# aanna0701/face-recognition-pytorch

Measured on AMD Instinct MI355X. Metric: train imgs/sec IR-50-layout ResNet50 + ArcFace/PartialFC head, 112x112, higher is better.
Workload: dtype bf16

## Files before the change

### face-recognition-pytorch_amd/frhip/build.py

```python
import hashlib
import os
import subprocess
import sys

HERE = os.path.dirname(os.path.abspath(__file__))
CSRC = os.path.join(HERE, "csrc")
ROOT = os.path.dirname(os.path.dirname(HERE))
LIB = os.path.join(HERE, "libfrhip.so")
SOURCES = ["misc.hip", "bn.hip", "stem.hip", "stem_fused.hip", "stem_algebra.hip", "igemm_nt.hip", "igemm_halo.hip", "igemm_tn.hip", "igemm_fp8.hip", "head.hip", "pfc_sample.hip", "margin.hip", "gallery_topk.hip", "winattn.hip", "winattn_mfma.hip", "cpb.hip", "optim.hip", "augment.hip"]
HIPCC = os.environ.get("HIPCC", "/opt/rocm/bin/hipcc")
FLAGS = ["--offload-arch=gfx950", "-O3", "-fPIC", "-std=c++17", "-munsafe-fp-atomics",
         "-I" + os.path.join(ROOT, "include"), "-I" + CSRC]
VARIANT = os.environ.get("FRHIP_VARIANT", "")
if VARIANT:
    FLAGS = FLAGS + os.environ.get("FRHIP_CXXFLAGS", "").split()
    LIB = os.path.join(HERE, "build", "var", "libfrhip_%s.so" % VARIANT)


def _digest(paths):
    h = hashlib.sha1(" ".join(FLAGS).replace(ROOT, "").encode())
    for p in sorted(paths):
        h.update(os.path.basename(p).encode())
        with open(p, "rb") as f:
            h.update(f.read())
    return h.hexdigest()


def _stale(target, deps):
    stamp = target + ".sha1"
    if not os.path.exists(target) or not os.path.exists(stamp):
        return True
    with open(stamp) as f:
        return f.read().strip() != _digest(deps)


def build(force=False, verbose=False):
    objdir = os.path.join(HERE, "build", "var", VARIANT) if VARIANT else os.path.join(HERE, "build")
    os.makedirs(objdir, exist_ok=True)
    headers = [os.path.join(CSRC, f) for f in os.listdir(CSRC) if f.endswith(".h")]
    headers.append(os.path.join(ROOT, "include", "frhip.h"))
    objs, procs = [], []
    for src in SOURCES:
        s = os.path.join(CSRC, src)
        o = os.path.join(objdir, src.replace(".hip", ".o"))
        objs.append(o)
        if force or _stale(o, [s] + headers):
            cmd = [HIPCC] + FLAGS + ["-c", s, "-o", o]
            if verbose:
                print(" ".join(cmd))
            procs.append((src, o, [s] + headers, subprocess.Popen(cmd, stdout=subprocess.PIPE, stderr=subprocess.STDOUT)))
    for src, o, deps, p in procs:
        out, _ = p.communicate()
        if p.returncode != 0:
            raise RuntimeError("hipcc failed on %s:\n%s" % (src, out.decode(errors="replace")))
        with open(o + ".sha1", "w") as f:
            f.write(_digest(deps))
    if force or procs or not os.path.exists(LIB):
        cmd = [HIPCC, "--offload-arch=gfx950", "-shared", "-fPIC", "-o", LIB] + objs
        r = subprocess.run(cmd, stdout=subprocess.PIPE, stderr=subprocess.STDOUT)
        if r.returncode != 0:
            raise RuntimeError("link failed:\n" + r.stdout.decode(errors="replace"))
    return LIB


if __name__ == "__main__":
    print(build(force="--force" in sys.argv, verbose=True))
```

### face-recognition-pytorch_amd/frhip/csrc/stem_algebra.hip

```cpp
#include "common.h"
#include "frhip.h"

namespace frhip {

constexpr int SG_ROWS = 8;
constexpr int SG_ROLES = 8;
constexpr int SG_VALS = 81;
constexpr int SG_OUT = 7 * SG_VALS;

template <typename T>
__global__ __launch_bounds__(256) void stem_gram_kernel(const float* __restrict__ x, float* __restrict__ partial, int B, int H, int W) {
    extern __shared__ __attribute__((aligned(16))) char smem[];
    float* xs = reinterpret_cast<float*>(smem);
    const int XR = SG_ROWS + 2, XC = W + 2;
    const int role = threadIdx.x & 7, pl = threadIdx.x >> 3;
    const int ca_ = role < 3 ? 0 : (role < 5 ? 1 : 2);
    const int cb_ = role < 3 ? role : (role < 5 ? role - 2 : 2);
    float acc[SG_VALS];
#pragma unroll
    for (int i = 0; i < SG_VALS; ++i) acc[i] = 0.f;
    const int bands = (H + SG_ROWS - 1) / SG_ROWS;
    for (int tile = blockIdx.x; tile < B * bands; tile += gridDim.x) {
        const int n = tile / bands, h0 = (tile - n * bands) * SG_ROWS;
        const float* ximg = x + (size_t)n * 3 * H * W;
        __syncthreads();
        for (int idx = threadIdx.x; idx < 3 * XR * XC; idx += 256) {
            const int cc = idx % XC, rest = idx / XC, rr = rest % XR, ci = rest / XR;
            const int h = h0 - 1 + rr, w = cc - 1;
            const float v = ((unsigned)h < (unsigned)H && (unsigned)w < (unsigned)W) ? ximg[((size_t)ci * H + h) * W + w] : 0.f;
            xs[idx] = to_f32<T>(from_f32<T>(v));
        }
        __syncthreads();
        const int rows = min(SG_ROWS, H - h0);
        for (int p = pl; p < rows * W; p += 32) {
            const int py = p / W, px = p - py * W;
            const float* base = xs + py * XC + px;
            if (role < 6) {
                float va[9], vb[9];
#pragma unroll
                for (int a = 0; a < 9; ++a) {
                    va[a] = base[(ca_ * XR + a / 3) * XC + a % 3];
                    vb[a] = base[(cb_ * XR + a / 3) * XC + a % 3];
                }
#pragma unroll
                for (int a = 0; a < 9; ++a)
#pragma unroll
                    for (int b = 0; b < 9; ++b) acc[a * 9 + b] = fmaf(va[a], vb[b], acc[a * 9 + b]);
            } else if (role == 6) {
#pragma unroll
                for (int c = 0; c < 3; ++c)
#pragma unroll
                    for (int a = 0; a < 9; ++a) acc[c * 9 + a] += base[(c * XR + a / 3) * XC + a % 3];
            }
        }
    }
    __syncthreads();
    float* red = reinterpret_cast<float*>(smem);
    const int lane = lane_id(), wave = wave_id();
#pragma unroll
    for (int i = 0; i < SG_VALS; ++i) {
        float v = acc[i];
        v = lane_sum_bit3(v); v = lane_sum_bit4(v); v = lane_sum_bit5(v);
        if (lane < 8) red[(wave * 8 + lane) * SG_VALS + i] = v;
    }
    __syncthreads();
    for (int o = threadIdx.x; o < SG_OUT; o += 256)
        partial[(size_t)blockIdx.x * SG_OUT + o] = red[o] + red[8 * SG_VALS + o] + red[16 * SG_VALS + o] + red[24 * SG_VALS + o];
}

__global__ __launch_bounds__(256) void stem_gram_fold_kernel(const float* __restrict__ partial, int nparts, float* __restrict__ blk) {
    __shared__ float red[3][SG_VALS];
    const int o = threadIdx.x % SG_VALS, part = threadIdx.x / SG_VALS;
    if (part < 3) {
        float a = 0.f;
        for (int p = part; p < nparts; p += 3) a += partial[(size_t)p * SG_OUT + blockIdx.x * SG_VALS + o];
        red[part][o] = a;
    }
    __syncthreads();
    if (threadIdx.x < SG_VALS) blk[blockIdx.x * SG_VALS + o] = red[0][o] + red[1][o] + red[2][o];
}

__global__ __launch_bounds__(256) void stem_gram_assemble_kernel(const float* __restrict__ blk, float* __restrict__ gram) {
    for (int o = threadIdx.x; o < 27 * 27 + 27; o += 256) {
        if (o < 729) {
            const int j = o / 27, j2 = o - j * 27;
            const int a = j / 3, c = j - a * 3, b = j2 / 3, c2 = j2 - b * 3;
            const int lo = c < c2 ? c : c2, hi = c < c2 ? c2 : c;
            const int role = lo == 0 ? hi : (lo == 1 ? 2 + hi : 5);
            gram[o] = c <= c2 ? blk[role * SG_VALS + a * 9 + b] : blk[role * SG_VALS + b * 9 + a];
        } else {
            const int j = o - 729, a = j / 3, c = j - a * 3;
            gram[o] = blk[6 * SG_VALS + c * 9 + a];
        }
    }
}

constexpr int DG_P = 8;
constexpr int DG_X = 2 * DG_P + 3;

template <typename T>
__global__ __launch_bounds__(256) void stem_dgather_kernel(const float* __restrict__ x, const T* __restrict__ dpool,
                                                           const T* __restrict__ pooled, const uint8_t* __restrict__ argmax,
                                                           float* __restrict__ slabs, int B, int H, int W) {
    __shared__ float xs[3 * DG_X * DG_X];
    __shared__ float gs[4 * 64 * 27];
    __shared__ uint8_t ab8[DG_P * DG_P * 64];
    const int Hp = (H - 1) / 2 + 1, Wp = (W - 1) / 2 + 1;
    const int th = (Hp + DG_P - 1) / DG_P, tw = (Wp + DG_P - 1) / DG_P;
    const int lane = lane_id(), wave = wave_id();
    float acc[27];
#pragma unroll
    for (int j = 0; j < 27; ++j) acc[j] = 0.f;
    constexpr int EPV = 16 / (int)sizeof(T), VPR = 64 / EPV;
    constexpr int XN = (3 * DG_X * DG_X + 255) / 256;
    constexpr int VN = DG_P * DG_P * VPR / 256;
    static_assert(DG_P * DG_P * VPR % 256 == 0, "tile vectors split evenly over the threads");
    float xr[XN];
    Vec16<T> gr[VN], pr[VN];
    uint64_t ar[VN];
    bool inr[VN];
    auto fetch = [&](int tile) {
        const int n = tile / (th * tw), rem = tile - n * th * tw;
        const int ph0 = (rem / tw) * DG_P, pw0 = (rem % tw) * DG_P;
        const float* ximg = x + (size_t)n * 3 * H * W;
#pragma unroll
        for (int i = 0; i < XN; ++i) {
            const int idx = threadIdx.x + i * 256;
            const int cc = idx % DG_X, rest = idx / DG_X, rr = rest % DG_X, ci = rest / DG_X;
            const int h = 2 * ph0 - 2 + rr, w = 2 * pw0 - 2 + cc;
            xr[i] = (idx < 3 * DG_X * DG_X && (unsigned)h < (unsigned)H && (unsigned)w < (unsigned)W) ? ximg[((size_t)ci * H + h) * W + w] : 0.f;
        }
#pragma unroll
        for (int i = 0; i < VN; ++i) {
            const int idx = threadIdx.x + i * 256;
            const int cv = idx % VPR, pp = idx / VPR, pl = pp / DG_P, pc = pp - pl * DG_P;
            const int ph = ph0 + pl, pw = pw0 + pc;
            inr[i] = ph < Hp && pw < Wp;
            const size_t o = ((((size_t)n * Hp + ph) * Wp + pw) * VPR + cv) * EPV;
            ar[i] = 0;
            if (inr[i]) {
                gr[i] = *reinterpret_cast<const Vec16<T>*>(dpool + o);
                pr[i] = *reinterpret_cast<const Vec16<T>*>(pooled + o);
                if constexpr (EPV == 8) ar[i] = *reinterpret_cast<const uint64_t*>(argmax + o);
                else ar[i] = *reinterpret_cast<const uint32_t*>(argmax + o);
            }
        }
    };
    const int ntiles = B * th * tw;
    if ((int)blockIdx.x < ntiles) fetch(blockIdx.x);
    for (int tile = blockIdx.x; tile < ntiles; tile += gridDim.x) {
        __syncthreads();
#pragma unroll
        for (int i = 0; i < XN; ++i) {
            const int idx = threadIdx.x + i * 256;
            if (idx < 3 * DG_X * DG_X) xs[idx] = to_f32<T>(from_f32<T>(xr[i]));
        }
#pragma unroll
        for (int i = 0; i < VN; ++i) {
            const int idx = threadIdx.x + i * 256;
            const int cv = idx % VPR, pp = idx / VPR;
#pragma unroll
            for (int e = 0; e < EPV; ++e) gs[pp * 64 + cv * EPV + e] = (inr[i] && pr[i].get(e) > 0.f) ? gr[i].get(e) : 0.f;
            if constexpr (EPV == 8) *reinterpret_cast<uint64_t*>(ab8 + pp * 64 + cv * 8) = ar[i];
            else *reinterpret_cast<uint32_t*>(ab8 + pp * 64 + cv * 4) = (uint32_t)ar[i];
        }
        __syncthreads();
        if (tile + (int)gridDim.x < ntiles) fetch(tile + gridDim.x);
        for (int pp = wave; pp < DG_P * DG_P; pp += 4) {
            const int pl = pp / DG_P, pc = pp - pl * DG_P;
            const float g = gs[pp * 64 + lane];
            const int a = ab8[pp * 64 + lane];
            const int r = (a * 11) >> 5, s = a - 3 * r;
            const float* base = xs + (2 * pl + r) * DG_X + 2 * pc + s;
#pragma unroll
            for (int t = 0; t < 9; ++t)
#pragma unroll
                for (int ci = 0; ci < 3; ++ci) acc[t * 3 + ci] = fmaf(g, base[(ci * DG_X + t / 3) * DG_X + t % 3], acc[t * 3 + ci]);
        }
    }
    __syncthreads();
    float* red = gs;
#pragma unroll
    for (int j = 0; j < 27; ++j) red[(wave * 64 + lane) * 27 + j] = acc[j];
    __syncthreads();
    for (int o = threadIdx.x; o < 64 * 32; o += 256) {
        const int k = o >> 5, j = o & 31;
        float a = 0.f;
        if (j < 27)
#pragma unroll
            for (int wv = 0; wv < 4; ++wv) a += red[(wv * 64 + k) * 27 + j];
        slabs[(size_t)blockIdx.x * 2048 + o] = a;
    }
}

template <typename T>
__global__ __launch_bounds__(1024) void stem_dw_final_kernel(const float* __restrict__ slabs, int nslabs, const float* __restrict__ gram,
                                                            const T* __restrict__ wp, const float* __restrict__ ca,
                                                            const float* __restrict__ cb, const float* __restrict__ cc,
                                                            float* __restrict__ dw) {
    __shared__ float red[32][32];
    const int k = blockIdx.x, j = threadIdx.x & 31, part = threadIdx.x >> 5;
    float a = 0.f;
    for (int s = part; s < nslabs; s += 32) a += slabs[(size_t)s * 2048 + k * 32 + j];
    red[part][j] = a;
    __syncthreads();
    if (threadIdx.x < 27) {
        float d = 0.f;
#pragma unroll
        for (int p = 0; p < 32; ++p) d += red[p][j];
        float wg = 0.f;
        for (int j2 = 0; j2 < 27; ++j2) wg = fmaf(to_f32<T>(wp[k * 32 + j2]), gram[j2 * 27 + j], wg);
        dw[k * 27 + j] += ca[k] * d + cb[k] * wg + cc[k] * gram[729 + j];
    }
}

}

using namespace frhip;

static bool sa_ok(int dtype, int b, int h, int w, const char* who) {
    if ((dtype != FRHIP_DT_BF16 && dtype != FRHIP_DT_F32) || b <= 0 || h <= 0 || w <= 0 || 3LL * b * h * w > 0x7fffffffLL ||
        3 * (SG_ROWS + 2) * (w + 2) * 4 > 60 * 1024) {
        set_error("%s: unsupported dtype / shape (dtype=%d b=%d h=%d w=%d)", who, dtype, b, h, w);
        return false;
    }
    return true;
}

extern "C" int frhip_stem_gram_floats(void) { return 27 * 27 + 27; }

extern "C" int frhip_stem_gram_blocks(int b, int h, int w) {
    const int t = b * ((h + SG_ROWS - 1) / SG_ROWS);
    return t < 512 ? t : 512;
}

extern "C" int frhip_stem_gram(int dtype, const float* x, int b, int h, int w, float* partial, float* gram, hipStream_t stream) {
    if (!sa_ok(dtype, b, h, w, "frhip_stem_gram")) return FRHIP_EINVAL;
    const int blocks = frhip_stem_gram_blocks(b, h, w);
    int lds = 3 * (SG_ROWS + 2) * (w + 2) * 4;
    if (lds < 4 * 8 * SG_VALS * 4) lds = 4 * 8 * SG_VALS * 4;
    if (dtype == FRHIP_DT_BF16) hipLaunchKernelGGL(stem_gram_kernel<bf16_t>, dim3(blocks), dim3(256), lds, stream, x, partial, b, h, w);
    else hipLaunchKernelGGL(stem_gram_kernel<float>, dim3(blocks), dim3(256), lds, stream, x, partial, b, h, w);
    int rc = check_launch("frhip_stem_gram");
    if (rc) return rc;
    float* blk = partial + (size_t)blocks * SG_OUT;
    hipLaunchKernelGGL(stem_gram_fold_kernel, dim3(7), dim3(256), 0, stream, partial, blocks, blk);
    hipLaunchKernelGGL(stem_gram_assemble_kernel, dim3(1), dim3(256), 0, stream, blk, gram);
    return check_launch("frhip_stem_gram(reduce)");
}

extern "C" int frhip_stem_bwd_wgrad_gram(int dtype, const float* x, const void* wp, const void* dpool, const void* pooled,
                                         const uint8_t* argmax, const float* gram, const float* ca, const float* cb, const float* cc,
                                         int b, int h, int w, float* slabs, float* dw, hipStream_t stream) {
    if (!sa_ok(dtype, b, h, w, "frhip_stem_bwd_wgrad_gram")) return FRHIP_EINVAL;
    const int blocks = frhip_stem_blocks(b, h, w);
    if (dtype == FRHIP_DT_BF16)
        hipLaunchKernelGGL(stem_dgather_kernel<bf16_t>, dim3(blocks), dim3(256), 0, stream, x, (const bf16_t*)dpool, (const bf16_t*)pooled,
                           argmax, slabs, b, h, w);
    else
        hipLaunchKernelGGL(stem_dgather_kernel<float>, dim3(blocks), dim3(256), 0, stream, x, (const float*)dpool, (const float*)pooled,
                           argmax, slabs, b, h, w);
    int rc = check_launch("frhip_stem_bwd_wgrad_gram(gather)");
    if (rc) return rc;
    if (dtype == FRHIP_DT_BF16)
        hipLaunchKernelGGL(stem_dw_final_kernel<bf16_t>, dim3(64), dim3(1024), 0, stream, slabs, blocks, gram, (const bf16_t*)wp, ca, cb, cc, dw);
    else
        hipLaunchKernelGGL(stem_dw_final_kernel<float>, dim3(64), dim3(1024), 0, stream, slabs, blocks, gram, (const float*)wp, ca, cb, cc, dw);
    return check_launch("frhip_stem_bwd_wgrad_gram(final)");
}
```

### face-recognition-pytorch_amd/frhip/csrc/stem_fused.hip

```cpp
#include "common.h"
#include "frhip.h"

namespace frhip {

constexpr int SF_PH = 4, SF_PW = 28;
constexpr int SF_RH = 2 * SF_PH + 1, SF_RW = 2 * SF_PW + 1;

template <typename T>
struct StemConv {
    static constexpr int EPL = 16 / (int)sizeof(T);
    static constexpr int RUNS = 32 / (4 * EPL);
    typedef typename Mma<T>::Frag Frag;
    Frag wf[RUNS][4];
    int koff[RUNS][EPL];
    const T* xs;
    int XR, XC;

    __device__ __forceinline__ void init(const T* __restrict__ wp, const T* xs_, int XR_, int XC_) {
        xs = xs_; XR = XR_; XC = XC_;
        const int lane = lane_id(), i = lane & 15, g = lane >> 4;
#pragma unroll
        for (int r = 0; r < RUNS; ++r) {
#pragma unroll
            for (int t = 0; t < 4; ++t)
                wf[r][t] = *reinterpret_cast<const Frag*>(wp + (t * 16 + i) * 32 + r * 4 * EPL + g * EPL);
#pragma unroll
            for (int e = 0; e < EPL; ++e) {
                const int k = r * 4 * EPL + g * EPL + e;
                const int tap = k / 3, ci = k - tap * 3, fr = tap / 3, fs = tap - fr * 3;
                koff[r][e] = k < 27 ? (ci * XR + fr) * XC + fs : 0;
            }
        }
    }
    __device__ __forceinline__ void stage(T* xs_w, const float* __restrict__ ximg, int h_org, int w_org, int H, int W) const {
        const int total = 3 * XR * XC;
        for (int idx = threadIdx.x; idx < total; idx += blockDim.x) {
            const int cc = idx % XC, rest = idx / XC;
            const int rr = rest % XR, ci = rest / XR;
            const int h = h_org + rr, w = w_org + cc;
            const float v = ((unsigned)h < (unsigned)H && (unsigned)w < (unsigned)W) ? ximg[((size_t)ci * H + h) * W + w] : 0.f;
            xs_w[idx] = from_f32<T>(v);
        }
    }
    __device__ __forceinline__ void gather(int hl, int wl, bool live, Frag (&b)[RUNS]) const {
        const int base = live ? hl * XC + wl : 0;
#pragma unroll
        for (int r = 0; r < RUNS; ++r) {
            Vec16<T> v;
#pragma unroll
            for (int e = 0; e < EPL; ++e) v.v[e] = xs[base + koff[r][e]];
            b[r] = v.v;
        }
    }
    __device__ __forceinline__ void conv(const Frag (&b)[RUNS], f32x4_t (&acc)[4]) const {
#pragma unroll
        for (int t = 0; t < 4; ++t) {
            acc[t] = f32x4_t{0.f, 0.f, 0.f, 0.f};
#pragma unroll
            for (int r = 0; r < RUNS; ++r) Mma<T>::run(wf[r][t], b[r], acc[t]);
        }
    }
};

template <int RB> __device__ __forceinline__ int sf_swz(int row);
template <> __device__ __forceinline__ int sf_swz<256>(int row) { return ((row & 3) << 2) | ((row >> 2) & 3); }
template <> __device__ __forceinline__ int sf_swz<128>(int row) { return (((row >> 1) & 1) | (((row >> 3) & 1) << 1)) << 1; }

template <typename T, int RB> struct SfFrag;
template <int RB> struct SfFrag<bf16_t, RB> {
    static constexpr int KROWS = 32;
    __device__ static __forceinline__ bf16x8_t load(const char* tile, int c0, int lane) {
        const int g = lane >> 4, j = lane & 15, q = j >> 2, p = j & 3;
        const int chunk = (c0 >> 3) + (p >> 1);
        const int row_a = 8 * g + q, row_b = row_a + 4;
        const char* pa = tile + row_a * RB + ((chunk ^ sf_swz<RB>(row_a)) << 4) + 8 * (p & 1);
        const char* pb = tile + row_b * RB + ((chunk ^ sf_swz<RB>(row_b)) << 4) + 8 * (p & 1);
        i16x4_t lo = __builtin_amdgcn_ds_read_tr16_b64_v4i16((__attribute__((address_space(3))) i16x4_t*)LDS_ADDR(pa));
        i16x4_t hi = __builtin_amdgcn_ds_read_tr16_b64_v4i16((__attribute__((address_space(3))) i16x4_t*)LDS_ADDR(pb));
        typedef __attribute__((ext_vector_type(8))) short i16x8_t;
        return __builtin_bit_cast(bf16x8_t, (i16x8_t)__builtin_shufflevector(lo, hi, 0, 1, 2, 3, 4, 5, 6, 7));
    }
};
template <int RB> struct SfFrag<float, RB> {
    static constexpr int KROWS = 16;
    __device__ static __forceinline__ f32x4_t load(const char* tile, int c0, int lane) {
        const int g = lane >> 4, i = lane & 15;
        const int col = c0 + i, chunk = col >> 2, within = (col & 3) * 4;
        f32x4_t v;
#pragma unroll
        for (int e = 0; e < 4; ++e) {
            const int row = 4 * e + g;
            v[e] = *reinterpret_cast<const float*>(tile + row * RB + ((chunk ^ sf_swz<RB>(row)) << 4) + within);
        }
        return v;
    }
};

__device__ __forceinline__ int sf_chan(int t, int reg) { return t * 16 + 4 * (lane_id() >> 4) + reg; }

__device__ __forceinline__ float sf_sum16(float v) { return lane_sum_row16(v); }

template <typename T>
__global__ __launch_bounds__(256) void stem_stats_kernel(const float* __restrict__ x, const T* __restrict__ wp,
                                                         float* __restrict__ partial, int B, int H, int W) {
    extern __shared__ __attribute__((aligned(16))) char smem[];
    T* xs = reinterpret_cast<T*>(smem);
    const int XR = 10, XC = W + 2;
    StemConv<T> sc;
    sc.init(wp, xs, XR, XC);
    const int lane = lane_id(), wave = wave_id(), i = lane & 15;
    const int bands = (H + 7) / 8;
    float s1[4][4], s2[4][4];
#pragma unroll
    for (int t = 0; t < 4; ++t)
#pragma unroll
        for (int r = 0; r < 4; ++r) { s1[t][r] = 0.f; s2[t][r] = 0.f; }
    for (int tile = blockIdx.x; tile < B * bands; tile += gridDim.x) {
        const int n = tile / bands, h0 = (tile - n * bands) * 8;
        __syncthreads();
        sc.stage(xs, x + (size_t)n * 3 * H * W, h0 - 1, -1, H, W);
        __syncthreads();
        for (int rr = 0; rr < 2; ++rr) {
            const int hl = wave * 2 + rr;
            if (h0 + hl >= H) break;
            for (int w0 = 0; w0 < W; w0 += 16) {
                const int w = w0 + i;
                typename StemConv<T>::Frag b[StemConv<T>::RUNS];
                f32x4_t acc[4];
                sc.gather(hl, w, w < W, b);
                sc.conv(b, acc);
#pragma unroll
                for (int t = 0; t < 4; ++t)
#pragma unroll
                    for (int r = 0; r < 4; ++r) { const float y = w < W ? acc[t][r] : 0.f; s1[t][r] += y; s2[t][r] += y * y; }
            }
        }
    }
    __syncthreads();
    float (*red)[2][64] = reinterpret_cast<float (*)[2][64]>(smem);
#pragma unroll
    for (int t = 0; t < 4; ++t)
#pragma unroll
        for (int r = 0; r < 4; ++r) {
            const float a = sf_sum16(s1[t][r]), b2 = sf_sum16(s2[t][r]);
            if (i == 0) { red[wave][0][sf_chan(t, r)] = a; red[wave][1][sf_chan(t, r)] = b2; }
        }
    __syncthreads();
    if (threadIdx.x < 128) {
        const int st = threadIdx.x >> 6, c = threadIdx.x & 63;
        partial[((size_t)blockIdx.x * 2 + st) * 64 + c] = red[0][st][c] + red[1][st][c] + red[2][st][c] + red[3][st][c];
    }
}

template <typename T>
__global__ __launch_bounds__(256) void stem_fwd_kernel(const float* __restrict__ x, const T* __restrict__ wp,
                                                       const float* __restrict__ scale, const float* __restrict__ shift,
                                                       T* __restrict__ pooled, uint8_t* __restrict__ argmax, int B, int H, int W) {
    constexpr int EPV = 16 / (int)sizeof(T), VPR = 64 / EPV;
    constexpr int PITCH = 64 * (int)sizeof(T) + 16;
    extern __shared__ __attribute__((aligned(16))) char smem[];
    constexpr int XR = SF_RH + 2, XC = SF_RW + 2;
    T* xs = reinterpret_cast<T*>(smem + SF_RH * SF_RW * PITCH);
    StemConv<T> sc;
    sc.init(wp, xs, XR, XC);
    const int lane = lane_id(), wave = wave_id(), i = lane & 15, g = lane >> 4;
    const int Hp = (H - 1) / 2 + 1, Wp = (W - 1) / 2 + 1;
    const int tw = (Wp + SF_PW - 1) / SF_PW, th = (Hp + SF_PH - 1) / SF_PH;
    int tile = blockIdx.x;
    const int n = tile / (tw * th); tile -= n * tw * th;
    const int ph0 = (tile / tw) * SF_PH, pw0 = (tile % tw) * SF_PW;
    sc.stage(xs, x + (size_t)n * 3 * H * W, 2 * ph0 - 2, 2 * pw0 - 2, H, W);
    __syncthreads();
    float sc_[4][4], sh_[4][4];
#pragma unroll
    for (int t = 0; t < 4; ++t)
#pragma unroll
        for (int r = 0; r < 4; ++r) { sc_[t][r] = scale[sf_chan(t, r)]; sh_[t][r] = shift[sf_chan(t, r)]; }
    for (int it = wave; it * 16 < SF_RH * SF_RW; it += 4) {
        const int rp = it * 16 + i;
        const int rr = rp / SF_RW, rc = rp - rr * SF_RW;
        const int h = 2 * ph0 - 1 + rr, w = 2 * pw0 - 1 + rc;
        const bool inside = rp < SF_RH * SF_RW && (unsigned)h < (unsigned)H && (unsigned)w < (unsigned)W;
        typename StemConv<T>::Frag b[StemConv<T>::RUNS];
        f32x4_t acc[4];
        sc.gather(rr, rc, rp < SF_RH * SF_RW, b);
        sc.conv(b, acc);
        if (rp < SF_RH * SF_RW) {
#pragma unroll
            for (int t = 0; t < 4; ++t) {
                T* dst = reinterpret_cast<T*>(smem + rp * PITCH) + t * 16 + 4 * g;
#pragma unroll
                for (int r = 0; r < 4; ++r) {
                    const float a = fmaxf(acc[t][r] * sc_[t][r] + sh_[t][r], 0.f);
                    dst[r] = from_f32<T>(inside ? a : -INFINITY);
                }
            }
        }
    }
    __syncthreads();
    for (int task = threadIdx.x; task < SF_PH * SF_PW * VPR; task += 256) {
        const int cv = task % VPR, pp = task / VPR;
        const int pl = pp / SF_PW, pc = pp - pl * SF_PW;
        const int ph = ph0 + pl, pw = pw0 + pc;
        if (ph >= Hp || pw >= Wp) continue;
        float best[EPV]; int bi[EPV];
#pragma unroll
        for (int e = 0; e < EPV; ++e) { best[e] = -INFINITY; bi[e] = 0; }
#pragma unroll
        for (int r = 0; r < 3; ++r)
#pragma unroll
            for (int s = 0; s < 3; ++s) {
                const Vec16<T> v = *reinterpret_cast<const Vec16<T>*>(smem + ((2 * pl + r) * SF_RW + 2 * pc + s) * PITCH + cv * 16);
#pragma unroll
                for (int e = 0; e < EPV; ++e) {
                    const float a = v.get(e);
                    if (a > best[e]) { best[e] = a; bi[e] = r * 3 + s; }
                }
            }
        const size_t o = ((((size_t)n * Hp + ph) * Wp + pw) * VPR + cv) * EPV;
        Vec16<T> ov;
#pragma unroll
        for (int e = 0; e < EPV; ++e) ov.set(e, best[e]);
        *reinterpret_cast<Vec16<T>*>(pooled + o) = ov;
        if constexpr (EPV == 8) {
            uint64_t pk = 0;
#pragma unroll
            for (int e = 0; e < 8; ++e) pk |= (uint64_t)(uint32_t)bi[e] << (8 * e);
            *reinterpret_cast<uint64_t*>(argmax + o) = pk;
        } else {
            uint32_t pk = 0;
#pragma unroll
            for (int e = 0; e < 4; ++e) pk |= (uint32_t)bi[e] << (8 * e);
            *reinterpret_cast<uint32_t*>(argmax + o) = pk;
        }
    }
}

template <typename T, bool WGRAD>
__global__ __launch_bounds__(256, 2) void stem_bwd_kernel(const float* __restrict__ x, const T* __restrict__ wp,
                                                       const T* __restrict__ dpool, const uint8_t* __restrict__ argmax,
                                                       const float* __restrict__ p0, const float* __restrict__ p1,
                                                       const float* __restrict__ p2, const float* __restrict__ scale,
                                                       const float* __restrict__ shift, float* __restrict__ outbuf,
                                                       int B, int H, int W) {
    constexpr int EPL = StemConv<T>::EPL, RUNS = StemConv<T>::RUNS;
    constexpr int TH = SF_PH + 1, TW = SF_PW + 1;
    constexpr int DROW = 64 * (int)sizeof(T) + 16;
    constexpr int AROW = 64 + 16;
    constexpr int DY_RB = 64 * (int)sizeof(T), COL_RB = 128;
    constexpr int KR = SfFrag<T, 128>::KROWS;
    constexpr int SUB = KR / 16;
    extern __shared__ __attribute__((aligned(16))) char smem[];
    char* s_dp = smem;
    uint8_t* s_arg = reinterpret_cast<uint8_t*>(smem + TH * TW * DROW);
    char* s_wg = smem + TH * TW * (DROW + AROW);
    constexpr int XR = 2 * SF_PH + 2, XC = 2 * SF_PW + 2;
    T* xs = reinterpret_cast<T*>(s_wg + (WGRAD ? 4 * KR * (DY_RB + COL_RB) : 0) + 5 * 64 * 4);
    StemConv<T> sc;
    sc.init(wp, xs, XR, XC);
    const int lane = lane_id(), wave = wave_id(), i = lane & 15, g = lane >> 4;
    char* my_dy = s_wg + wave * KR * (DY_RB + COL_RB);
    char* my_col = my_dy + KR * DY_RB;
    const int Hp = (H - 1) / 2 + 1, Wp = (W - 1) / 2 + 1;
    const int tw = (Wp + SF_PW - 1) / SF_PW, th = (Hp + SF_PH - 1) / SF_PH;
    float* s_const = reinterpret_cast<float*>(s_wg + (WGRAD ? 4 * KR * (DY_RB + COL_RB) : 0));
    for (int v = threadIdx.x; v < 64; v += 256) {
        s_const[v] = scale[v]; s_const[64 + v] = shift[v];
        if (WGRAD) { s_const[128 + v] = p0[v]; s_const[192 + v] = p1[v]; s_const[256 + v] = p2[v]; }
    }
    auto cvec = [&](int which, int t) { return *reinterpret_cast<const f32x4_t*>(s_const + which * 64 + t * 16 + 4 * g); };
    float s1[4][4], s2[4][4];
    f32x4_t dw[4][2];
#pragma unroll
    for (int t = 0; t < 4; ++t) {
#pragma unroll
        for (int r = 0; r < 4; ++r) { s1[t][r] = 0.f; s2[t][r] = 0.f; }
        dw[t][0] = f32x4_t{0.f, 0.f, 0.f, 0.f}; dw[t][1] = dw[t][0];
    }
    if (WGRAD && sizeof(T) == 2) {
        for (int v = lane; v < KR * COL_RB / 16; v += 64) *reinterpret_cast<f32x4_t*>(my_col + v * 16) = f32x4_t{0.f, 0.f, 0.f, 0.f};
    }

    for (int tile = blockIdx.x; tile < B * th * tw; tile += gridDim.x) {
        int rem = tile;
        const int n = rem / (tw * th); rem -= n * tw * th;
        const int ph0 = (rem / tw) * SF_PH, pw0 = (rem % tw) * SF_PW;
        __syncthreads();
        sc.stage(xs, x + (size_t)n * 3 * H * W, 2 * ph0 - 1, 2 * pw0 - 1, H, W);
        constexpr int VPT = 64 * (int)sizeof(T) / 16;
        for (int v = threadIdx.x; v < TH * TW * VPT; v += 256) {
            const int pix = v / VPT, part = v - pix * VPT;
            const int ph = ph0 + pix / TW, pw = pw0 + pix % TW;
            f32x4_t val = f32x4_t{0.f, 0.f, 0.f, 0.f};
            if (ph < Hp && pw < Wp)
                val = *reinterpret_cast<const f32x4_t*>(reinterpret_cast<const char*>(dpool) +
                                                        ((((size_t)n * Hp + ph) * Wp + pw) * 64) * sizeof(T) + part * 16);
            *reinterpret_cast<f32x4_t*>(s_dp + pix * DROW + part * 16) = val;
        }
        for (int v = threadIdx.x; v < TH * TW * 4; v += 256) {
            const int pix = v >> 2, part = v & 3;
            const int ph = ph0 + pix / TW, pw = pw0 + pix % TW;
            f32x4_t val = f32x4_t{0.f, 0.f, 0.f, 0.f};
            if (ph < Hp && pw < Wp)
                val = *reinterpret_cast<const f32x4_t*>(argmax + (((size_t)n * Hp + ph) * Wp + pw) * 64 + part * 16);
            *reinterpret_cast<f32x4_t*>(s_arg + pix * AROW + part * 16) = val;
        }
        __syncthreads();
        for (int grp = wave; grp * KR < 4 * SF_PH * SF_PW; grp += 4) {
#pragma unroll
            for (int sub = 0; sub < SUB; ++sub) {
                const int bp = grp * KR + sub * 16 + i;
                const int br = bp / (2 * SF_PW), bc = bp - br * (2 * SF_PW);
                const int h = 2 * ph0 + br, w = 2 * pw0 + bc;
                const bool live = bp < 4 * SF_PH * SF_PW && h < H && w < W;
                typename StemConv<T>::Frag b[RUNS];
                f32x4_t acc[4];
                sc.gather(br, bc, bp < 4 * SF_PH * SF_PW, b);
                sc.conv(b, acc);
                float d[4][4];
#pragma unroll
                for (int t = 0; t < 4; ++t)
#pragma unroll
                    for (int r = 0; r < 4; ++r) d[t][r] = 0.f;
                const int plo = (h >> 1) - ph0, phi = ((h + 1) >> 1) - ph0, qlo = (w >> 1) - pw0, qhi = ((w + 1) >> 1) - pw0;
#pragma unroll 1
                for (int pp = 0; pp < 2; ++pp) {
                    const int pl = pp == 0 ? plo : phi;
                    const bool rowuse = live && (pp == 0 || phi != plo) && ph0 + pl < Hp;
                    const int rtap = (h - (2 * (ph0 + pl) - 1)) * 3;
#pragma unroll
                    for (int qq = 0; qq < 2; ++qq) {
                        const int pc = qq == 0 ? qlo : qhi;
                        const bool use = rowuse && (qq == 0 || qhi != qlo) && pw0 + pc < Wp;
                        const int tap = rtap + (w - (2 * (pw0 + pc) - 1));
                        const int pix = use ? pl * TW + pc : 0;
#pragma unroll
                        for (int t = 0; t < 4; ++t) {
                            const int ch0 = t * 16 + 4 * g;
                            const uint32_t a4 = *reinterpret_cast<const uint32_t*>(s_arg + pix * AROW + ch0);
                            float dv[4];
                            if constexpr (sizeof(T) == 2) {
                                const bf16x4_t q = *reinterpret_cast<const bf16x4_t*>(s_dp + pix * DROW + ch0 * 2);
#pragma unroll
                                for (int r = 0; r < 4; ++r) dv[r] = (float)q[r];
                            } else {
                                const f32x4_t q = *reinterpret_cast<const f32x4_t*>(s_dp + pix * DROW + ch0 * 4);
#pragma unroll
                                for (int r = 0; r < 4; ++r) dv[r] = q[r];
                            }
#pragma unroll
                            for (int r = 0; r < 4; ++r)
                                if (use && (int)((a4 >> (8 * r)) & 0xffu) == tap) d[t][r] += dv[r];
                        }
                    }
                }
#pragma unroll
                for (int t = 0; t < 4; ++t) {
                    const f32x4_t ms = cvec(0, t), mb = cvec(1, t);
                    f32x4_t ca, cb, cc;
                    if (WGRAD) { ca = cvec(2, t); cb = cvec(3, t); cc = cvec(4, t); }
#pragma unroll
                    for (int r = 0; r < 4; ++r) {
                        const float y = acc[t][r];
                        const float de = (live && y * ms[r] + mb[r] > 0.f) ? d[t][r] : 0.f;
                        if (WGRAD) d[t][r] = live ? ca[r] * de + cb[r] * y + cc[r] : 0.f;
                        else { s1[t][r] += de; s2[t][r] += de * y; }
                    }
                }
                if (WGRAD) {
                    const int row = sub * 16 + i;
#pragma unroll
                    for (int t = 0; t < 4; ++t) {
                        constexpr int CPV = 16 / (int)sizeof(T);
                        const int ch0 = t * 16 + 4 * g;
                        char* dst = my_dy + row * DY_RB + (((ch0 / CPV) ^ sf_swz<DY_RB>(row)) << 4) + (ch0 % CPV) * (int)sizeof(T);
                        if constexpr (sizeof(T) == 2) {
                            bf16x4_t q;
#pragma unroll
                            for (int r = 0; r < 4; ++r) q[r] = (bf16_t)d[t][r];
                            *reinterpret_cast<bf16x4_t*>(dst) = q;
                        } else {
                            *reinterpret_cast<f32x4_t*>(dst) = f32x4_t{d[t][0], d[t][1], d[t][2], d[t][3]};
                        }
                    }
#pragma unroll
                    for (int rn = 0; rn < RUNS; ++rn) {
                        const int chunk = rn * 4 + g;
                        *reinterpret_cast<typename StemConv<T>::Frag*>(my_col + row * COL_RB + ((chunk ^ sf_swz<COL_RB>(row)) << 4)) = b[rn];
                    }
                }
            }
            if (WGRAD) {
                typename StemConv<T>::Frag af[4], bf[2];
#pragma unroll
                for (int t = 0; t < 4; ++t) af[t] = SfFrag<T, DY_RB>::load(my_dy, t * 16, lane);
#pragma unroll
                for (int kt = 0; kt < 2; ++kt) bf[kt] = SfFrag<T, COL_RB>::load(my_col, kt * 16, lane);
#pragma unroll
                for (int t = 0; t < 4; ++t)
#pragma unroll
                    for (int kt = 0; kt < 2; ++kt) Mma<T>::run(af[t], bf[kt], dw[t][kt]);
            }
        }
    }
    __syncthreads();
    if (!WGRAD) {
        float (*red)[2][64] = reinterpret_cast<float (*)[2][64]>(smem);
#pragma unroll
        for (int t = 0; t < 4; ++t)
#pragma unroll
            for (int r = 0; r < 4; ++r) {
                const float a = sf_sum16(s1[t][r]), b2 = sf_sum16(s2[t][r]);
                if (i == 0) { red[wave][0][sf_chan(t, r)] = a; red[wave][1][sf_chan(t, r)] = b2; }
            }
        __syncthreads();
        if (threadIdx.x < 64) {
            const int c = threadIdx.x;
            const float sd = red[0][0][c] + red[1][0][c] + red[2][0][c] + red[3][0][c];
            const float sdy = red[0][1][c] + red[1][1][c] + red[2][1][c] + red[3][1][c];
            outbuf[((size_t)blockIdx.x * 2 + 0) * 64 + c] = sd;
            outbuf[((size_t)blockIdx.x * 2 + 1) * 64 + c] = p1[c] * (sdy - p0[c] * sd);
        }
    } else {
        float* red = reinterpret_cast<float*>(smem);
#pragma unroll
        for (int t = 0; t < 4; ++t)
#pragma unroll
            for (int kt = 0; kt < 2; ++kt)
#pragma unroll
                for (int r = 0; r < 4; ++r) red[(wave * 64 + t * 16 + 4 * g + r) * 32 + kt * 16 + i] = dw[t][kt][r];
        __syncthreads();
        for (int o = threadIdx.x; o < 64 * 32; o += 256)
            outbuf[(size_t)blockIdx.x * 2048 + o] = red[o] + red[2048 + o] + red[4096 + o] + red[6144 + o];
    }
}

constexpr int SB_THREADS = 512, SB_WAVES = 8;
constexpr int SB_NPIX = 4 * SF_PH * SF_PW;
constexpr int SB_TH = SF_PH + 1, SB_TW = SF_PW + 1;
constexpr int SB_DROW = 128 + 16, SB_AROW = 64 + 16;
constexpr int SB_OFF_ARG = SB_TH * SB_TW * SB_DROW;
constexpr int SB_OFF_XS = SB_OFF_ARG + SB_TH * SB_TW * SB_AROW;
constexpr int SB_XR = 2 * SF_PH + 2, SB_XC = 2 * SF_PW + 2;
constexpr int SB_OFF_CONST = SB_OFF_XS + ((3 * SB_XR * SB_XC * 2 + 15) / 16) * 16;
constexpr int SB_OFF_TILE = SB_OFF_CONST + 5 * 64 * 4;
constexpr int SB_OFF_MASK = SB_OFF_TILE + SB_NPIX * 128;
constexpr int SB_OFF_COL = SB_OFF_MASK + SB_NPIX * 8;
constexpr int SB_LDS_REDUCE = SB_OFF_MASK > SB_THREADS * 16 * 4 ? SB_OFF_MASK : SB_THREADS * 16 * 4;
constexpr int SB_LDS_WGRAD = SB_OFF_COL + SB_WAVES * 32 * 128;

__device__ __forceinline__ int sb_addr(int row, int c) { return row * 128 + (((c >> 3) ^ sf_swz<128>(row)) << 4) + (c & 7) * 2; }

template <bool WGRAD>
__global__ __launch_bounds__(SB_THREADS, 1) void stem_bwd2_kernel(const float* __restrict__ x, const bf16_t* __restrict__ wp,
                                                                 const bf16_t* __restrict__ dpool, const uint8_t* __restrict__ argmax,
                                                                 const float* __restrict__ p0, const float* __restrict__ p1,
                                                                 const float* __restrict__ p2, const float* __restrict__ scale,
                                                                 const float* __restrict__ shift, float* __restrict__ outbuf,
                                                                 int B, int H, int W) {
    typedef bf16_t T;
    extern __shared__ __attribute__((aligned(16))) char smem[];
    char* s_dp = smem;
    uint8_t* s_arg = reinterpret_cast<uint8_t*>(smem + SB_OFF_ARG);
    T* xs = reinterpret_cast<T*>(smem + SB_OFF_XS);
    float* s_const = reinterpret_cast<float*>(smem + SB_OFF_CONST);
    char* s_tile = smem + SB_OFF_TILE;
    uint32_t* s_mask = reinterpret_cast<uint32_t*>(smem + SB_OFF_MASK);
    StemConv<T> sc;
    sc.init(wp, xs, SB_XR, SB_XC);
    const int lane = lane_id(), wave = wave_id(), i = lane & 15, g = lane >> 4;
    char* my_col = smem + SB_OFF_COL + wave * 32 * 128;
    const int Hp = (H - 1) / 2 + 1, Wp = (W - 1) / 2 + 1;
    const int tw = (Wp + SF_PW - 1) / SF_PW, th = (Hp + SF_PH - 1) / SF_PH;
    for (int v = threadIdx.x; v < 64; v += SB_THREADS) {
        s_const[v] = scale[v]; s_const[64 + v] = shift[v];
        if (WGRAD) { s_const[128 + v] = p0[v]; s_const[192 + v] = p1[v]; s_const[256 + v] = p2[v]; }
    }
    auto cvec = [&](int which, int t) { return *reinterpret_cast<const f32x4_t*>(s_const + which * 64 + t * 16 + 4 * g); };
    const int cv = threadIdx.x & 7;
    float s1[8], s2[8];
#pragma unroll
    for (int e = 0; e < 8; ++e) { s1[e] = 0.f; s2[e] = 0.f; }
    f32x4_t dw[4][2];
#pragma unroll
    for (int t = 0; t < 4; ++t) { dw[t][0] = f32x4_t{0.f, 0.f, 0.f, 0.f}; dw[t][1] = dw[t][0]; }
    if (WGRAD)
        for (int v = lane; v < 32 * 128 / 16; v += 64) *reinterpret_cast<f32x4_t*>(my_col + v * 16) = f32x4_t{0.f, 0.f, 0.f, 0.f};

    for (int tile = blockIdx.x; tile < B * th * tw; tile += gridDim.x) {
        int rem = tile;
        const int n = rem / (tw * th); rem -= n * tw * th;
        const int ph0 = (rem / tw) * SF_PH, pw0 = (rem % tw) * SF_PW;
        __syncthreads();
        sc.stage(xs, x + (size_t)n * 3 * H * W, 2 * ph0 - 1, 2 * pw0 - 1, H, W);
        for (int v = threadIdx.x; v < SB_TH * SB_TW * 8; v += SB_THREADS) {
            const int pix = v >> 3, part = v & 7;
            const int ph = ph0 + pix / SB_TW, pw = pw0 + pix % SB_TW;
            f32x4_t val = f32x4_t{0.f, 0.f, 0.f, 0.f};
            if (ph < Hp && pw < Wp)
                val = *reinterpret_cast<const f32x4_t*>(reinterpret_cast<const char*>(dpool) + ((((size_t)n * Hp + ph) * Wp + pw) * 64) * 2 + part * 16);
            *reinterpret_cast<f32x4_t*>(s_dp + pix * SB_DROW + part * 16) = val;
        }
        for (int v = threadIdx.x; v < SB_TH * SB_TW * 4; v += SB_THREADS) {
            const int pix = v >> 2, part = v & 3;
            const int ph = ph0 + pix / SB_TW, pw = pw0 + pix % SB_TW;
            f32x4_t val = f32x4_t{0.f, 0.f, 0.f, 0.f};
            if (ph < Hp && pw < Wp)
                val = *reinterpret_cast<const f32x4_t*>(argmax + (((size_t)n * Hp + ph) * Wp + pw) * 64 + part * 16);
            *reinterpret_cast<f32x4_t*>(s_arg + pix * SB_AROW + part * 16) = val;
        }
        if (WGRAD) for (int v = threadIdx.x; v < SB_NPIX * 2; v += SB_THREADS) s_mask[v] = 0u;
        __syncthreads();
        for (int it = wave; it * 16 < SB_NPIX; it += SB_WAVES) {
            const int bp = it * 16 + i;
            const int br = bp / (2 * SF_PW), bc = bp - br * (2 * SF_PW);
            const bool live = 2 * ph0 + br < H && 2 * pw0 + bc < W;
            typename StemConv<T>::Frag b[1];
            f32x4_t acc[4];
            sc.gather(br, bc, true, b);
            sc.conv(b, acc);
            uint32_t mbits[2] = {0u, 0u};
#pragma unroll
            for (int t = 0; t < 4; ++t) {
                const int ch0 = t * 16 + 4 * g;
                bf16x4_t q;
                if (WGRAD) {
                    const f32x4_t ms = cvec(0, t), mb = cvec(1, t), cb = cvec(3, t), cc = cvec(4, t);
#pragma unroll
                    for (int r = 0; r < 4; ++r) {
                        const float y = acc[t][r];
                        q[r] = (bf16_t)(live ? cb[r] * y + cc[r] : 0.f);
                        if (live && y * ms[r] + mb[r] > 0.f) mbits[ch0 >> 5] |= 1u << ((ch0 & 31) + r);
// ... 499 lines not shown
```

Baseline: 23380.

## Use MFMA for stem Gram, vectorise stem staging, bit-trick maxpool, cache build

Replaces the scalar FMA stem Gram-matrix kernel for bf16 with an MFMA kernel that stages three shifted bf16 copies of the input window and accumulates 32x32 outer products, with a ones column for the channel sums. Adds a shared row-wise, paired-load staging helper used by several stem kernels. The fused stem forward now packs bf16 values with a tap index into integers so the 3x3 maxpool and its argmax come from integer max operations, and skips the border masking on interior tiles. The stats kernel gets a fast path for full column groups, and the build script skips rebuilding when the library digest is unchanged. These changes target the stem's ALU and staging cost, at the price of more complex code and a larger LDS footprint for the Gram kernel.

```diff
diff --git a/face-recognition-pytorch_amd/frhip/build.py b/face-recognition-pytorch_amd/frhip/build.py
--- a/face-recognition-pytorch_amd/frhip/build.py
+++ b/face-recognition-pytorch_amd/frhip/build.py
@@ -39,6 +39,9 @@
     os.makedirs(objdir, exist_ok=True)
     headers = [os.path.join(CSRC, f) for f in os.listdir(CSRC) if f.endswith(".h")]
     headers.append(os.path.join(ROOT, "include", "frhip.h"))
+    all_inputs = [os.path.join(CSRC, s) for s in SOURCES] + headers
+    if not force and not _stale(LIB, all_inputs):
+        return LIB
     objs, procs = [], []
     for src in SOURCES:
         s = os.path.join(CSRC, src)
@@ -60,6 +63,8 @@
         r = subprocess.run(cmd, stdout=subprocess.PIPE, stderr=subprocess.STDOUT)
         if r.returncode != 0:
             raise RuntimeError("link failed:\n" + r.stdout.decode(errors="replace"))
+    with open(LIB + ".sha1", "w") as f:
+        f.write(_digest(all_inputs))
     return LIB
 
 
diff --git a/face-recognition-pytorch_amd/frhip/csrc/stem_algebra.hip b/face-recognition-pytorch_amd/frhip/csrc/stem_algebra.hip
--- a/face-recognition-pytorch_amd/frhip/csrc/stem_algebra.hip
+++ b/face-recognition-pytorch_amd/frhip/csrc/stem_algebra.hip
@@ -1,5 +1,6 @@
 #include "common.h"
 #include "frhip.h"
+#include "stem_stage.h"
 
 namespace frhip {
 
@@ -24,12 +25,7 @@
         const int n = tile / bands, h0 = (tile - n * bands) * SG_ROWS;
         const float* ximg = x + (size_t)n * 3 * H * W;
         __syncthreads();
-        for (int idx = threadIdx.x; idx < 3 * XR * XC; idx += 256) {
-            const int cc = idx % XC, rest = idx / XC, rr = rest % XR, ci = rest / XR;
-            const int h = h0 - 1 + rr, w = cc - 1;
-            const float v = ((unsigned)h < (unsigned)H && (unsigned)w < (unsigned)W) ? ximg[((size_t)ci * H + h) * W + w] : 0.f;
-            xs[idx] = to_f32<T>(from_f32<T>(v));
-        }
+        stem_stage<T, float>(xs, ximg, h0 - 1, -1, H, W, XR, XC);
         __syncthreads();
         const int rows = min(SG_ROWS, H - h0);
         for (int p = pl; p < rows * W; p += 32) {
@@ -66,6 +62,79 @@
     __syncthreads();
     for (int o = threadIdx.x; o < SG_OUT; o += 256)
         partial[(size_t)blockIdx.x * SG_OUT + o] = red[o] + red[8 * SG_VALS + o] + red[16 * SG_VALS + o] + red[24 * SG_VALS + o];
+}
+
+constexpr int SGM_RED = 4 * 32 * 32 * 4;
+__device__ __host__ inline int sgm_cols(int W) { return (W + 31) & ~31; }
+__device__ __host__ inline int sgm_pitch(int W) { return sgm_cols(W) + 8; }
+__device__ __host__ inline int sgm_lds(int W) {
+    const int win = 3 * 3 * (SG_ROWS + 2) * sgm_pitch(W) * 2;
+    return win > SGM_RED ? win : SGM_RED;
+}
+
+__global__ __launch_bounds__(256) void stem_gram_mfma_kernel(const float* __restrict__ x, float* __restrict__ partial, int B, int H, int W) {
+    extern __shared__ __attribute__((aligned(16))) char smem[];
+    bf16_t* xs = reinterpret_cast<bf16_t*>(smem);
+    constexpr int XR = SG_ROWS + 2;
+    const int XC = W + 2, XP = sgm_pitch(W), CS = 3 * XR * XP;
+    const int ncg = sgm_cols(W) >> 5;
+    const int lane = lane_id(), wave = wave_id(), i = lane & 15, g = lane >> 4;
+    for (int v = threadIdx.x; v < 3 * CS / 8; v += 256) *reinterpret_cast<f32x4_t*>(smem + v * 16) = f32x4_t{0.f, 0.f, 0.f, 0.f};
+    int off[2];
+#pragma unroll
+    for (int t = 0; t < 2; ++t) {
+        const int j = t * 16 + i;
+        const int c = j / 9, tap = j - c * 9, fr = tap / 3, fs = tap - fr * 3;
+        off[t] = j < 27 ? fs * CS + (c * XR + fr) * XP + 8 * g : 8 * g;
+    }
+    const bf16_t one = (bf16_t)1.f, zero = (bf16_t)0.f;
+    bf16x8_t ones_full, ones_last;
+#pragma unroll
+    for (int e = 0; e < 8; ++e) {
+        ones_full[e] = i == 11 ? one : zero;
+        ones_last[e] = (i == 11 && (ncg - 1) * 32 + 8 * g + e < W) ? one : zero;
+    }
+    f32x4_t d00 = {0.f, 0.f, 0.f, 0.f}, d01 = d00, d11 = d00;
+    const int bands = (H + SG_ROWS - 1) / SG_ROWS;
+    for (int tile = blockIdx.x; tile < B * bands; tile += gridDim.x) {
+        const int n = tile / bands, h0 = (tile - n * bands) * SG_ROWS;
+        __syncthreads();
+        stem_stage_copies<bf16_t, bf16_t, 3>(xs, x + (size_t)n * 3 * H * W, h0 - 1, -1, H, W, XR, XC, XP, CS, W);
+        __syncthreads();
+        const int rows = min(SG_ROWS, H - h0);
+        for (int ks = wave; ks < rows * ncg; ks += 4) {
+            const int py = ks / ncg, cg = ks - py * ncg;
+            const bf16_t* base = xs + py * XP + cg * 32;
+            const bf16x8_t f0 = *reinterpret_cast<const bf16x8_t*>(base + off[0]);
+            bf16x8_t f1 = *reinterpret_cast<const bf16x8_t*>(base + off[1]);
+            if (i >= 11) f1 = cg == ncg - 1 ? ones_last : ones_full;
+            d00 = __builtin_amdgcn_mfma_f32_16x16x32_bf16(f0, f0, d00, 0, 0, 0);
+            d01 = __builtin_amdgcn_mfma_f32_16x16x32_bf16(f0, f1, d01, 0, 0, 0);
+            d11 = __builtin_amdgcn_mfma_f32_16x16x32_bf16(f1, f1, d11, 0, 0, 0);
+        }
+    }
+    __syncthreads();
+    float* red = reinterpret_cast<float*>(smem);
+#pragma unroll
+    for (int r = 0; r < 4; ++r) {
+        red[(wave * 32 + 4 * g + r) * 32 + i] = d00[r];
+        red[(wave * 32 + 4 * g + r) * 32 + 16 + i] = d01[r];
+        red[(wave * 32 + 16 + 4 * g + r) * 32 + 16 + i] = d11[r];
+    }
+    __syncthreads();
+    for (int o = threadIdx.x; o < SG_OUT; o += 256) {
+        const int role = o / SG_VALS, rem = o - role * SG_VALS, a = rem / 9, b = rem - a * 9;
+        int j, j2;
+        if (role < 6) {
+            const int c = role < 3 ? 0 : (role < 5 ? 1 : 2), c2 = role < 3 ? role : (role < 5 ? role - 2 : 2);
+            j = c * 9 + a; j2 = c2 * 9 + b;
+            if (j > j2) { const int t = j; j = j2; j2 = t; }
+        } else {
+            j = rem; j2 = 27;
+        }
+        const int e = j * 32 + j2;
+        partial[(size_t)blockIdx.x * SG_OUT + o] = red[e] + red[1024 + e] + red[2048 + e] + red[3072 + e];
+    }
 }
 
 __global__ __launch_bounds__(256) void stem_gram_fold_kernel(const float* __restrict__ partial, int nparts, float* __restrict__ blk) {
@@ -237,10 +306,16 @@
 extern "C" int frhip_stem_gram(int dtype, const float* x, int b, int h, int w, float* partial, float* gram, hipStream_t stream) {
     if (!sa_ok(dtype, b, h, w, "frhip_stem_gram")) return FRHIP_EINVAL;
     const int blocks = frhip_stem_gram_blocks(b, h, w);
-    int lds = 3 * (SG_ROWS + 2) * (w + 2) * 4;
-    if (lds < 4 * 8 * SG_VALS * 4) lds = 4 * 8 * SG_VALS * 4;
-    if (dtype == FRHIP_DT_BF16) hipLaunchKernelGGL(stem_gram_kernel<bf16_t>, dim3(blocks), dim3(256), lds, stream, x, partial, b, h, w);
-    else hipLaunchKernelGGL(stem_gram_kernel<float>, dim3(blocks), dim3(256), lds, stream, x, partial, b, h, w);
+    if (dtype == FRHIP_DT_BF16) {
+        const int lds = sgm_lds(w);
+        if (lds > 64 * 1024 && set_dynamic_lds(reinterpret_cast<const void*>(stem_gram_mfma_kernel), 160 * 1024, "frhip_stem_gram"))
+            return FRHIP_ELAUNCH;
+        hipLaunchKernelGGL(stem_gram_mfma_kernel, dim3(blocks), dim3(256), lds, stream, x, partial, b, h, w);
+    } else {
+        int lds = 3 * (SG_ROWS + 2) * (w + 2) * 4;
+        if (lds < 4 * 8 * SG_VALS * 4) lds = 4 * 8 * SG_VALS * 4;
+        hipLaunchKernelGGL(stem_gram_kernel<float>, dim3(blocks), dim3(256), lds, stream, x, partial, b, h, w);
+    }
     int rc = check_launch("frhip_stem_gram");
     if (rc) return rc;
     float* blk = partial + (size_t)blocks * SG_OUT;
diff --git a/face-recognition-pytorch_amd/frhip/csrc/stem_fused.hip b/face-recognition-pytorch_amd/frhip/csrc/stem_fused.hip
--- a/face-recognition-pytorch_amd/frhip/csrc/stem_fused.hip
+++ b/face-recognition-pytorch_amd/frhip/csrc/stem_fused.hip
@@ -1,5 +1,6 @@
 #include "common.h"
 #include "frhip.h"
+#include "stem_stage.h"
 
 namespace frhip {
 
@@ -33,14 +34,7 @@
         }
     }
     __device__ __forceinline__ void stage(T* xs_w, const float* __restrict__ ximg, int h_org, int w_org, int H, int W) const {
-        const int total = 3 * XR * XC;
-        for (int idx = threadIdx.x; idx < total; idx += blockDim.x) {
-            const int cc = idx % XC, rest = idx / XC;
-            const int rr = rest % XR, ci = rest / XR;
-            const int h = h_org + rr, w = w_org + cc;
-            const float v = ((unsigned)h < (unsigned)H && (unsigned)w < (unsigned)W) ? ximg[((size_t)ci * H + h) * W + w] : 0.f;
-            xs_w[idx] = from_f32<T>(v);
-        }
+        stem_stage<T, T>(xs_w, ximg, h_org, w_org, H, W, XR, XC);
     }
     __device__ __forceinline__ void gather(int hl, int wl, bool live, Frag (&b)[RUNS]) const {
         const int base = live ? hl * XC + wl : 0;
@@ -100,6 +94,15 @@
 
 __device__ __forceinline__ float sf_sum16(float v) { return lane_sum_row16(v); }
 
+__device__ __forceinline__ float sf_sq_acc(int e, float y, float s2) {
+    if (e < 10) return __builtin_fmaf(y, y, s2);
+    {
+#pragma clang fp contract(off)
+        const float q = y * y;
+        return q + s2;
+    }
+}
+
 template <typename T>
 __global__ __launch_bounds__(256) void stem_stats_kernel(const float* __restrict__ x, const T* __restrict__ wp,
                                                          float* __restrict__ partial, int B, int H, int W) {
@@ -129,10 +132,17 @@
                 f32x4_t acc[4];
                 sc.gather(hl, w, w < W, b);
                 sc.conv(b, acc);
-#pragma unroll
-                for (int t = 0; t < 4; ++t)
-#pragma unroll
-                    for (int r = 0; r < 4; ++r) { const float y = w < W ? acc[t][r] : 0.f; s1[t][r] += y; s2[t][r] += y * y; }
+                if (w0 + 16 <= W) {
+#pragma unroll
+                    for (int t = 0; t < 4; ++t)
+#pragma unroll
+                        for (int r = 0; r < 4; ++r) { const float y = acc[t][r]; s1[t][r] += y; s2[t][r] = sf_sq_acc(t * 4 + r, y, s2[t][r]); }
+                } else {
+#pragma unroll
+                    for (int t = 0; t < 4; ++t)
+#pragma unroll
+                        for (int r = 0; r < 4; ++r) { const float y = w < W ? acc[t][r] : 0.f; s1[t][r] += y; s2[t][r] = sf_sq_acc(t * 4 + r, y, s2[t][r]); }
+                }
             }
         }
     }
@@ -156,7 +166,6 @@
 __global__ __launch_bounds__(256) void stem_fwd_kernel(const float* __restrict__ x, const T* __restrict__ wp,
                                                        const float* __restrict__ scale, const float* __restrict__ shift,
                                                        T* __restrict__ pooled, uint8_t* __restrict__ argmax, int B, int H, int W) {
-    constexpr int EPV = 16 / (int)sizeof(T), VPR = 64 / EPV;
     constexpr int PITCH = 64 * (int)sizeof(T) + 16;
     extern __shared__ __attribute__((aligned(16))) char smem[];
     constexpr int XR = SF_RH + 2, XC = SF_RW + 2;
@@ -185,49 +194,77 @@
         f32x4_t acc[4];
         sc.gather(rr, rc, rp < SF_RH * SF_RW, b);
         sc.conv(b, acc);
+        const int ra = (it * 16) / SF_RW, rb = (it * 16 + 15) / SF_RW, ca = it * 16 - ra * SF_RW;
+        const int wl = 2 * pw0 - 1 + (ra == rb ? ca : 0), wr = 2 * pw0 - 1 + (ra == rb ? ca + 15 : SF_RW - 1);
+        const bool interior = it * 16 + 15 < SF_RH * SF_RW && 2 * ph0 - 1 + ra >= 0 && 2 * ph0 - 1 + rb < H && wl >= 0 && wr < W;
         if (rp < SF_RH * SF_RW) {
 #pragma unroll
             for (int t = 0; t < 4; ++t) {
                 T* dst = reinterpret_cast<T*>(smem + rp * PITCH) + t * 16 + 4 * g;
-#pragma unroll
-                for (int r = 0; r < 4; ++r) {
-                    const float a = fmaxf(acc[t][r] * sc_[t][r] + sh_[t][r], 0.f);
-                    dst[r] = from_f32<T>(inside ? a : -INFINITY);
+                float a[4];
+#pragma unroll
+                for (int r = 0; r < 4; ++r) a[r] = fmaxf(acc[t][r] * sc_[t][r] + sh_[t][r], 0.f);
+                if constexpr (sizeof(T) == 2) {
+                    typedef __attribute__((ext_vector_type(4))) short i16x4v;
+                    i16x4v q = __builtin_bit_cast(i16x4v, bf16x4_t{(bf16_t)a[0], (bf16_t)a[1], (bf16_t)a[2], (bf16_t)a[3]});
+                    q = __builtin_elementwise_max(q, i16x4v{0, 0, 0, 0});
+                    if (!interior) {
+#pragma unroll
+                        for (int r = 0; r < 4; ++r) q[r] = inside ? q[r] : (short)0xFF80;
+                    }
+                    *reinterpret_cast<i16x4v*>(dst) = q;
+                } else {
+                    if (!interior) {
+#pragma unroll
+                        for (int r = 0; r < 4; ++r) a[r] = inside ? a[r] : -INFINITY;
+                    }
+                    *reinterpret_cast<f32x4_t*>(dst) = f32x4_t{a[0], a[1], a[2], a[3]};
                 }
             }
         }
     }
     __syncthreads();
-    for (int task = threadIdx.x; task < SF_PH * SF_PW * VPR; task += 256) {
-        const int cv = task % VPR, pp = task / VPR;
+    for (int task = threadIdx.x; task < SF_PH * SF_PW * 16; task += 256) {
+        const int cq = task & 15, pp = task >> 4;
         const int pl = pp / SF_PW, pc = pp - pl * SF_PW;
         const int ph = ph0 + pl, pw = pw0 + pc;
         if (ph >= Hp || pw >= Wp) continue;
-        float best[EPV]; int bi[EPV];
-#pragma unroll
-        for (int e = 0; e < EPV; ++e) { best[e] = -INFINITY; bi[e] = 0; }
-#pragma unroll
-        for (int r = 0; r < 3; ++r)
-#pragma unroll
-            for (int s = 0; s < 3; ++s) {
-                const Vec16<T> v = *reinterpret_cast<const Vec16<T>*>(smem + ((2 * pl + r) * SF_RW + 2 * pc + s) * PITCH + cv * 16);
-#pragma unroll
-                for (int e = 0; e < EPV; ++e) {
-                    const float a = v.get(e);
-                    if (a > best[e]) { best[e] = a; bi[e] = r * 3 + s; }
-                }
-            }
-        const size_t o = ((((size_t)n * Hp + ph) * Wp + pw) * VPR + cv) * EPV;
-        Vec16<T> ov;
-#pragma unroll
-        for (int e = 0; e < EPV; ++e) ov.set(e, best[e]);
-        *reinterpret_cast<Vec16<T>*>(pooled + o) = ov;
-        if constexpr (EPV == 8) {
-            uint64_t pk = 0;
-#pragma unroll
-            for (int e = 0; e < 8; ++e) pk |= (uint64_t)(uint32_t)bi[e] << (8 * e);
-            *reinterpret_cast<uint64_t*>(argmax + o) = pk;
+        const char* win = smem + ((2 * pl) * SF_RW + 2 * pc) * PITCH + cq * 4 * (int)sizeof(T);
+        const size_t o = (((size_t)n * Hp + ph) * Wp + pw) * 64 + cq * 4;
+        if constexpr (sizeof(T) == 2) {
+            int best[4];
+#pragma unroll
+            for (int tap = 0; tap < 9; ++tap) {
+                const u32x2_t d = *reinterpret_cast<const u32x2_t*>(win + ((tap / 3) * SF_RW + tap % 3) * PITCH);
+                const uint32_t c = 15u - (uint32_t)tap;
+                const int k[4] = {(int)((d[0] << 16) | c), (int)((d[0] & 0xffff0000u) | c), (int)((d[1] << 16) | c),
+                                  (int)((d[1] & 0xffff0000u) | c)};
+#pragma unroll
+                for (int e = 0; e < 4; ++e) best[e] = tap == 0 ? k[e] : max(best[e], k[e]);
+            }
+            u32x2_t ov;
+            ov[0] = ((uint32_t)best[0] >> 16) | ((uint32_t)best[1] & 0xffff0000u);
+            ov[1] = ((uint32_t)best[2] >> 16) | ((uint32_t)best[3] & 0xffff0000u);
+            *reinterpret_cast<u32x2_t*>(pooled + o) = ov;
+            const uint32_t low = ((uint32_t)best[0] & 15u) | (((uint32_t)best[1] & 15u) << 8) | (((uint32_t)best[2] & 15u) << 16) |
+                                 (((uint32_t)best[3] & 15u) << 24);
+            *reinterpret_cast<uint32_t*>(argmax + o) = 0x0f0f0f0fu - low;
         } else {
+            float best[4]; int bi[4];
+#pragma unroll
+            for (int e = 0; e < 4; ++e) { best[e] = -INFINITY; bi[e] = 0; }
+#pragma unroll
+            for (int r = 0; r < 3; ++r)
+#pragma unroll
+                for (int s = 0; s < 3; ++s) {
+                    const f32x4_t v = *reinterpret_cast<const f32x4_t*>(win + (r * SF_RW + s) * PITCH);
+#pragma unroll
+                    for (int e = 0; e < 4; ++e) {
+                        const float a = v[e];
+                        if (a > best[e]) { best[e] = a; bi[e] = r * 3 + s; }
+                    }
+                }
+            *reinterpret_cast<f32x4_t*>(pooled + o) = f32x4_t{best[0], best[1], best[2], best[3]};
             uint32_t pk = 0;
 #pragma unroll
             for (int e = 0; e < 4; ++e) pk |= (uint32_t)bi[e] << (8 * e);
diff --git a/face-recognition-pytorch_amd/frhip/csrc/stem_stage.h b/face-recognition-pytorch_amd/frhip/csrc/stem_stage.h
--- /dev/null
+++ b/face-recognition-pytorch_amd/frhip/csrc/stem_stage.h
@@ -0,0 +1,60 @@
+#pragma once
+#include <type_traits>
+
+#include "common.h"
+
+namespace frhip {
+
+template <typename T, typename ST> __device__ __forceinline__ ST stem_stage_value(float v) {
+    if constexpr (std::is_same<T, ST>::value) return from_f32<T>(v);
+    else return (ST)to_f32<T>(from_f32<T>(v));
+}
+
+template <typename T, typename ST, int NCOPY>
+__device__ __forceinline__ void stem_stage_copies(ST* __restrict__ xs, const float* __restrict__ ximg, int h_org, int w_org, int H, int W,
+                                                  int XR, int XC, int pitch, int copy_stride, int climit) {
+    const int lane = lane_id(), wave = wave_id(), nwaves = (int)(blockDim.x >> 6);
+    const int off = w_org & 1;
+    const int P = (XC + off + 1) >> 1;
+    int lsh = 6;
+    while (lsh > 3 && (1 << (lsh - 1)) >= P) --lsh;
+    const int lpr = 1 << lsh, rpw = 64 >> lsh;
+    const int sub = lane >> lsh, pl = lane & (lpr - 1);
+    const bool wide = !(W & 1) && !(reinterpret_cast<uintptr_t>(ximg) & 7);
+    const int rows = 3 * XR;
+    for (int q0 = wave * rpw; q0 < rows; q0 += nwaves * rpw) {
+        const int q = q0 + sub;
+        if (q >= rows) continue;
+        const int ci = q / XR, h = h_org + q - ci * XR;
+        const bool hin = (unsigned)h < (unsigned)H;
+        const float* src = ximg + ((size_t)ci * H + (hin ? h : 0)) * W;
+        ST* dst = xs + q * pitch;
+        for (int p = pl; p < P; p += lpr) {
+            const int cc = 2 * p - off, w = w_org + cc;
+            float v0 = 0.f, v1 = 0.f;
+            if (hin) {
+                if (wide) {
+                    if ((unsigned)w < (unsigned)W) { const f32x2_t t = *reinterpret_cast<const f32x2_t*>(src + w); v0 = t[0]; v1 = t[1]; }
+                } else {
+                    if ((unsigned)w < (unsigned)W) v0 = src[w];
+                    if ((unsigned)(w + 1) < (unsigned)W) v1 = src[w + 1];
+                }
+            }
+            const ST s0 = stem_stage_value<T, ST>(v0), s1 = stem_stage_value<T, ST>(v1);
+#pragma unroll
+            for (int s = 0; s < NCOPY; ++s) {
+                const int c = cc - s;
+                if (cc < XC && (unsigned)c < (unsigned)climit) dst[s * copy_stride + c] = s0;
+                if (cc + 1 < XC && (unsigned)(c + 1) < (unsigned)climit) dst[s * copy_stride + c + 1] = s1;
+            }
+        }
+    }
+}
+
+template <typename T, typename ST>
+__device__ __forceinline__ void stem_stage(ST* __restrict__ xs, const float* __restrict__ ximg, int h_org, int w_org, int H, int W,
+                                           int XR, int XC) {
+    stem_stage_copies<T, ST, 1>(xs, ximg, h_org, w_org, H, W, XR, XC, XC, 0, XC);
+}
+
+}
```

New measurement: 23580 (median of 6 runs). No clear change (+0.8%).
